# TUMFTM/ORB_SLAM3_RGBL

Hardware: AMD Instinct MI355X
Metric: RGB-L front-end frames/sec (extract+depth+match) (higher is better)
Workload: dtype u8; 1 GPU; KITTI-00 RGB-L cfg2 (synthetic stand-in); nfeatures=2000, levels=8, lidar_points=121600, match=Hamming brute force, frame i vs i+1, upsampling=InverseDilation Diamond 5, inputs=resident in HBM, parallelism=frames/sequences sharded, 1 rank(s), gather=none

## Files before the change

### orb_slam3_rgbl_amd/csrc/extractor.hip

```cpp
#include <math.h>
#include <stdarg.h>
#include <stdlib.h>
#include <string.h>

#include <algorithm>
#include <vector>

#include "brief_pattern.h"
#include "extractor_kernels.h"
#include "octree_labels.h"

namespace rgbl {

static thread_local char g_err[512] = "";
void set_error(const char* fmt, ...) {
  va_list ap;
  va_start(ap, fmt);
  vsnprintf(g_err, sizeof(g_err), fmt, ap);
  va_end(ap);
}
const char* last_error() { return g_err; }

static inline int round_even_f(float v) { return (int)lrintf(v); }
static inline int round_even_d(double v) { return (int)lrint(v); }
// ... 111 lines not shown
    t.a0 = (int16_t)round_even_f((1.f - f) * 2048);
    t.a1 = (int16_t)round_even_f(f * 2048);
    tab.push_back(t);
  }
}

int build_geometry(rgbl_extractor* e) {
  const rgbl_extractor_cfg& c = e->cfg;
  const int L = c.nlevels;
  e->L = L;
  e->scale.assign(L, 1.f); e->sigma2.assign(L, 1.f); e->inv_scale.assign(L, 1.f); e->inv_sigma2.assign(L, 1.f);
  for (int i = 1; i < L; ++i) {
    e->scale[i] = e->scale[i - 1] * c.scale_factor;
    e->sigma2[i] = e->scale[i] * e->scale[i];
  }
  for (int i = 0; i < L; ++i) {
    e->inv_scale[i] = 1.0f / e->scale[i];
    e->inv_sigma2[i] = 1.0f / e->sigma2[i];
  }
  e->per_level.assign(L, 0);
  const float factor = 1.0f / c.scale_factor;
  float desired = c.nfeatures * (1 - factor) / (1 - (float)pow((double)factor, (double)L));
  int sum = 0;
  for (int l = 0; l < L - 1; ++l) {
    e->per_level[l] = round_even_f(desired);
    sum += e->per_level[l];
    desired *= factor;
  }
  e->per_level[L - 1] = std::max(c.nfeatures - sum, 0);
  {
    int* u = e->umax.v;
    for (int i = 0; i < 16; ++i) u[i] = 0;
    const int vmax = floor_f(15 * sqrtf(2.f) / 2 + 1), vmin = ceil_f(15 * sqrtf(2.f) / 2);
    for (int v = 0; v <= vmax; ++v) u[v] = round_even_d(sqrt(225.0 - v * v));
    for (int v = 15, v0 = 0; v >= vmin; --v) {
      while (u[v0] == u[v0 + 1]) ++v0;
      u[v] = v0;
      ++v0;
    }
  }
  e->geom.assign(L, LevelGeom());
  size_t img_off = 0, slot_off = 0, node_off = 0, rootx_off = 0, xtab_off = 0, ytab_off = 0;
  int cell_off = 0, koff = 0;
  e->img_pitch = (int)align_up(c.width, 64);
  e->img_frame = (size_t)e->img_pitch * c.height;
  int tile_off = 0;
  for (int l = 0; l < L; ++l) {
    LevelGeom& g = e->geom[l];
    memset(&g, 0, sizeof(g));
    g.w = round_even_f((float)c.width * e->inv_scale[l]);
    g.h = round_even_f((float)c.height * e->inv_scale[l]);
    g.pitch = (int)align_up(g.w, 64);
    g.img_off = (uint32_t)img_off;
    img_off += (size_t)g.pitch * g.h;
    g.quota = e->per_level[l];
    g.scale = e->scale[l];
    g.patch_size = (int)(31 * e->scale[l]);
    g.max_bx = g.w - 19 + 3;
    g.max_by = g.h - 19 + 3;
    const float width = (float)(g.max_bx - kMinBorder), height = (float)(g.max_by - kMinBorder);
    g.n_cols = (int)(width / 35.f);
    g.n_rows = (int)(height / 35.f);
    if (g.n_cols < 1 || g.n_rows < 1) {
      set_error("level %d (%dx%d) is smaller than one 35-px detection cell; the reference divides by zero here", l, g.w, g.h);
      return RGBL_ERR_INVALID;
    }
    g.w_cell = (int)ceilf(width / g.n_cols);
    g.h_cell = (int)ceilf(height / g.n_rows);
    if (g.w_cell > kCellMax || g.h_cell > kCellMax) {
      set_error("cell %dx%d exceeds the kernel tile", g.w_cell, g.h_cell);
      return RGBL_ERR_INVALID;
    }
    e->max_cell = std::max(e->max_cell, std::max(g.w_cell, g.h_cell));
    e->max_cell_w = std::max(e->max_cell_w, g.w_cell);
    g.n_cells = g.n_cols * g.n_rows;
    g.m_wcell = (0x100000u + (uint32_t)g.w_cell - 1u) / (uint32_t)g.w_cell;
    g.m_hcell = (0x100000u + (uint32_t)g.h_cell - 1u) / (uint32_t)g.h_cell;
    g.cell_off = cell_off;
    cell_off += g.n_cells;
    g.cell_cap = ((g.w_cell + 1) / 2) * ((g.h_cell + 1) / 2);
    g.slot_off = (uint32_t)slot_off;
    g.key_off = (uint32_t)slot_off;
    g.key_cap = (uint32_t)((size_t)g.n_cells * g.cell_cap);
    slot_off += (size_t)g.n_cells * g.cell_cap;
    g.n_ini = (int)roundf((float)(g.max_bx - kMinBorder) / (float)(g.max_by - kMinBorder));
    if (g.n_ini < 1 || g.n_ini > kMaxRoots) {
      set_error("aspect ratio gives %d quad-tree roots (supported 1..%d; the reference fails for portrait images)", g.n_ini, kMaxRoots);
      return RGBL_ERR_INVALID;
    }
    const float hX = (float)(g.max_bx - kMinBorder) / g.n_ini;
    for (int i = 0; i <= g.n_ini; ++i) g.root_x[i] = (int)(hX * (float)i);
    g.rootx_off = (uint32_t)rootx_off;
    rootx_off += align_up((size_t)(g.max_bx - kMinBorder) + 1, 16);
    g.kcap = std::max(g.quota, 4 * g.n_ini) + 8;
    g.koff = koff;
    koff += g.kcap;
    g.node_cap = (uint32_t)g.kcap + 16;
    if (g.node_cap > 65535u) {
      set_error("nfeatures too large: level %d would need %u quad-tree nodes (limit 65535)", l, g.node_cap);
      return RGBL_ERR_INVALID;
    }
    g.node_off = (uint32_t)node_off;
    node_off += g.node_cap;
    g.xtab_off = (uint32_t)xtab_off;
    g.ytab_off = (uint32_t)ytab_off;
    if (l > 0) { xtab_off += align_up(g.w, 4); ytab_off += g.h; }
    e->blur_tiles.tile_off[l] = tile_off;
// ... 304 lines not shown
      RGBL_HIP(hipStreamWaitEvent(ls, e->ev_r, 0));
      launch_fast(ls, cells0, e->geom[k].cell_off);
      launch_octree(ls, 1, k);
      RGBL_HIP(hipEventRecord(e->ev_fb, ls));
      for (int l = k; l < L; ++l) launch_resize(s, l);
      RGBL_HIP(hipEventRecord(e->ev_pyr, s));
      launch_fast(s, e->geom[k].cell_off, e->cells_frame);
      launch_octree(s, k, L);
      RGBL_HIP(hipStreamWaitEvent(bs, e->ev_pyr, 0));
      launch_gauss(bs, tiles0, e->blur_tiles.tile_off[L]);
      RGBL_HIP(hipEventRecord(e->ev_blur, bs));
      RGBL_HIP(hipStreamWaitEvent(s, e->ev_fb, 0));
      RGBL_HIP(hipStreamWaitEvent(s, e->ev_fast0, 0));
      RGBL_HIP(hipStreamWaitEvent(s, e->ev_blur, 0));
    } else {
    if (overlap) {
      RGBL_HIP(hipEventRecord(e->ev_start, s));
      RGBL_HIP(hipStreamWaitEvent(bs, e->ev_start, 0));
      launch_fast(bs, 0, cells0);
      launch_gauss(bs, 0, tiles0);
      launch_octree(bs, 0, 1);
      RGBL_HIP(hipEventRecord(e->ev_fast0, bs));
    }
    for (int l = 1; l < L; ++l) launch_resize(s, l);
    if (overlap) {
      RGBL_HIP(hipEventRecord(e->ev_pyr, s));
      RGBL_HIP(hipStreamWaitEvent(bs, e->ev_pyr, 0));
      launch_gauss(bs, tiles0, e->blur_tiles.tile_off[L]);
      RGBL_HIP(hipEventRecord(e->ev_blur, bs));
    } else {
      launch_gauss(s, 0, e->blur_tiles.tile_off[L]);
    }
    if (overlap) {
      launch_fast(s, cells0, e->cells_frame);
    } else {
      launch_fast(s, 0, e->cells_frame);
    }
    if (overlap) {
      launch_octree(s, 1, L);
      RGBL_HIP(hipStreamWaitEvent(s, e->ev_fast0, 0));
    } else {
      launch_octree(s, 0, L);
    }
    if (overlap) RGBL_HIP(hipStreamWaitEvent(s, e->ev_blur, 0));
    }
  }
  const bool lapping = lap1 >= 19 && lap1 >= lap0;
  rgbl_keypoint* kp_dst = lapping ? e->d_tmp_kp : d_kp;
  uint8_t* desc_dst = lapping ? e->d_tmp_desc : d_desc;
  int lap_cap = cap;
  if (lapping) lap_cap = std::min(cap, e->out_cap);
  const bool split_desc = !e->timer.enabled && batch >= 8 && L > 1 && e->geom[1].koff > 0;
  const int slot_split = split_desc ? e->geom[1].koff : 0;
  auto launch_desc = [&](hipStream_t st, int slot_begin, int slot_end, int write_total) {
    if (slot_end <= slot_begin) return;
    e->timer.begin("k_orient_brief", st);
    hipLaunchKernelGGL(k_orient_brief<256>, xcd_grid(e->xcd_map, (slot_end - slot_begin + 4 * kKpPerWave - 1) / (4 * kKpPerWave), batch), dim3(256), 0, st, e->d_geom, L, e->umax,
                       e->d_pattern, d_imgs, stride, frame_stride, e->d_pyr, e->pyr_frame, e->d_blur, e->pyr_frame,
                       e->d_kpkey, e->d_kpcount, (size_t)e->kp_frame, kp_dst, desc_dst, lapping ? e->out_cap : cap, d_n,
                       lapping ? (int32_t*)nullptr : d_mono, e->d_err, slot_begin, slot_end, write_total);
    e->timer.end(st);
  };
  if (split_desc) {
    launch_desc(e->aux_stream, 0, slot_split, 0);
    RGBL_HIP(hipEventRecord(e->ev_desc0, e->aux_stream));
  }
  launch_desc(s, slot_split, e->kp_frame, 1);
  if (split_desc) RGBL_HIP(hipStreamWaitEvent(s, e->ev_desc0, 0));
  if (lapping) {
    (void)lap_cap;
    if (cap < e->out_cap) {
      set_error("vLappingArea packing needs cap >= %d", e->out_cap);
      return RGBL_ERR_CAPACITY;
    }
    e->timer.begin("k_lapping_permute", s);
    hipLaunchKernelGGL(k_lapping_permute, dim3(batch), dim3(256), 0, s, e->d_tmp_kp, e->d_tmp_desc, e->out_cap, d_kp,
                       d_desc, cap, d_n, (float)lap0, (float)lap1, d_mono);
    e->timer.end(s);
  }
  RGBL_HIP(hipGetLastError());
  e->dense_dirty = false;
  return RGBL_OK;
}

int check_device_flags(rgbl_extractor* e) {
  int flags = 0;
  RGBL_HIP(hipMemcpy(&flags, e->d_err, sizeof(int), hipMemcpyDeviceToHost));
  if (flags) {
    RGBL_HIP(hipMemset(e->d_err, 0, sizeof(int)));
    RGBL_HIP(hipMemset(e->d_levelcnt, 0, sizeof(uint32_t) * (size_t)e->cfg.max_batch * e->L));
    if (flags & 3) { set_error("quad-tree scratch overflow (flags=%d)", flags); return RGBL_ERR_OVERFLOW; }
    set_error("more keypoints than the caller's capacity");
    return RGBL_ERR_CAPACITY;
  }
  return RGBL_OK;
}

}

extern "C" {

const char* rgbl_last_error(void) { return rgbl::last_error(); }
const char* rgbl_backend(void) {
#ifdef RGBL_EMU
  return "emu";
#else
  return "hip:gfx950";
#endif
}
int rgbl_device_count(void) {
  int n = 0;
  if (hipGetDeviceCount(&n) != hipSuccess) return 0;
  return n;
// ... 422 lines not shown
  return RGBL_OK;
}

int rgbl_extract_color(rgbl_extractor* e, const uint8_t* img, int channels, int blue_first, int w, int h, int stride, int lap0,
                       int lap1, rgbl_keypoint* out_kp, uint8_t* out_desc, int cap, int* out_n, int* out_mono,
                       uint8_t* out_gray, int gray_stride) {
  if (out_n) *out_n = 0;
  if (out_mono) *out_mono = -1;
  if (!e) { set_error("null handle"); return RGBL_ERR_INVALID; }
  if (!img || w <= 0 || h <= 0) { set_error("empty image"); return RGBL_ERR_EMPTY; }
  if (!out_kp || !out_desc || !out_n || !out_mono) { set_error("null output"); return RGBL_ERR_INVALID; }
  if (channels == 1) {
    if (out_gray) for (int y = 0; y < h; ++y) memcpy(out_gray + (size_t)y * gray_stride, img + (size_t)y * stride, w);
    return rgbl_extract(e, img, w, h, stride, lap0, lap1, out_kp, out_desc, cap, out_n, out_mono);
  }
  if ((channels != 3 && channels != 4) || w != e->cfg.width || h != e->cfg.height || stride < w * channels || cap < 1 ||
      (out_gray && gray_stride < w)) {
    set_error("colour image %dx%dx%d does not match the handle (%dx%d)", w, h, channels, e->cfg.width, e->cfg.height);
    return RGBL_ERR_INVALID;
  }
  RGBL_HIP(hipSetDevice(e->device));
  RGBL_TRY(drop_pending(e));
  hipStream_t s = e->stream;
  const size_t need = (size_t)stride * h + 16;
  if (need > e->color_bytes) {
    if (e->d_color) RGBL_HIP(hipFree(e->d_color));
    e->d_color = nullptr; e->color_bytes = 0;
    RGBL_HIP(hipMalloc(&e->d_color, need));
    e->color_bytes = need;
  }
  RGBL_HIP(hipMemcpyAsync(e->d_color, img, (size_t)(h - 1) * stride + (size_t)w * channels, hipMemcpyHostToDevice, s));
  RGBL_TRY(enqueue_cvt_gray(e, (const uint8_t*)e->d_color, 1, channels, blue_first, w, h, stride, 0, e->d_img, e->img_pitch, 0));
  if (out_gray) RGBL_HIP(hipMemcpy2DAsync(out_gray, gray_stride, e->d_img, e->img_pitch, w, h, hipMemcpyDeviceToHost, s));
  return run_staged(e, 1, e->img_pitch, lap0, lap1, out_kp, out_desc, cap, out_n, out_mono);
}

int rgbl_extractor_level_size(const rgbl_extractor* e, int level, int* w, int* h) {
  if (!e || level < 0 || level >= e->L) { set_error("bad level"); return RGBL_ERR_INVALID; }
  if (w) *w = e->geom[level].w;
  if (h) *h = e->geom[level].h;
  return RGBL_OK;
}

int rgbl_extractor_get_level(rgbl_extractor* e, int frame, int level, int blurred, int with_border, uint8_t* dst,
                             int dst_stride) {
  if (!e || !dst || level < 0 || level >= e->L || frame < 0 || frame >= e->last_batch) {
    set_error("bad level/frame");
    return RGBL_ERR_INVALID;
  }
  RGBL_HIP(hipSetDevice(e->device));
  const LevelGeom& g = e->geom[level];
  const uint8_t* src;
  int pitch;
  if (blurred) { src = e->d_blur + (size_t)frame * e->pyr_frame + g.img_off; pitch = g.pitch; }
  else if (level == 0) { src = e->last_img0 + (size_t)frame * e->last_frame0; pitch = e->last_pitch0; }
  else { src = e->d_pyr + (size_t)frame * e->pyr_frame + g.img_off; pitch = g.pitch; }
  const int border = (with_border && !blurred) ? 19 : 0;
  RGBL_HIP(hipStreamSynchronize(e->stream));
  uint8_t* inner = dst + (size_t)border * dst_stride + border;
  {
    std::vector<uint8_t> tmp((size_t)pitch * (g.h - 1) + g.w);
    RGBL_HIP(hipMemcpyAsync(tmp.data(), src, tmp.size(), hipMemcpyDeviceToHost, e->stream));
    RGBL_HIP(hipStreamSynchronize(e->stream));
    for (int y = 0; y < g.h; ++y) memcpy(inner + (size_t)y * dst_stride, tmp.data() + (size_t)y * pitch, g.w);
  }
  if (border) {
    auto refl = [](int p, int len) { while (p < 0 || p >= len) p = p < 0 ? -p : 2 * (len - 1) - p; return p; };
    for (int y = 0; y < g.h; ++y) {
      uint8_t* row = inner + (size_t)y * dst_stride;
      for (int x = 1; x <= border; ++x) { row[-x] = row[refl(-x, g.w)]; row[g.w - 1 + x] = row[refl(g.w - 1 + x, g.w)]; }
    }
    for (int y = 1; y <= border; ++y) {
      memcpy(inner + (ptrdiff_t)(-y) * dst_stride - border, inner + (ptrdiff_t)refl(-y, g.h) * dst_stride - border, g.w + 2 * border);
      memcpy(inner + (ptrdiff_t)(g.h - 1 + y) * dst_stride - border, inner + (ptrdiff_t)refl(g.h - 1 + y, g.h) * dst_stride - border,
             g.w + 2 * border);
    }
  }
  return RGBL_OK;
}

int rgbl_extractor_get_candidates(rgbl_extractor* e, int frame, int level, rgbl_keypoint* out, int cap, int* out_n) {
  if (!e || level < 0 || level >= e->L || frame < 0 || frame >= e->last_batch || !out_n) {
    set_error("bad level/frame");
    return RGBL_ERR_INVALID;
  }
  RGBL_HIP(hipSetDevice(e->device));
  RGBL_HIP(hipStreamSynchronize(e->stream));
  const LevelGeom& g = e->geom[level];
  auto emit = [&](uint32_t key, int n) {
    if (out && n < cap) {
      rgbl_keypoint kp;
      kp.x = (float)(key & 0xfff); kp.y = (float)((key >> 12) & 0xfff); kp.size = 7.f; kp.angle = -1.f;
      kp.response = (float)(key >> 24); kp.octave = 0; kp.class_id = -1;
      out[n] = kp;
    }
  };
  int n = 0;
  if (e->dense) {
    uint32_t C = 0;
    RGBL_HIP(hipMemcpy(&C, e->d_levelcnt + ((size_t)e->cfg.max_batch + frame) * e->L + level, sizeof(uint32_t), hipMemcpyDeviceToHost));
    C = std::min(C, g.key_cap);
    std::vector<uint32_t> keys(C);
    if (C) RGBL_HIP(hipMemcpy(keys.data(), e->d_keys_a + (size_t)frame * e->keys_frame + g.key_off, sizeof(uint32_t) * C, hipMemcpyDeviceToHost));
    auto order = [&](uint32_t key) {
      const uint32_t x = (key & 0xfff) - 3u, y = ((key >> 12) & 0xfff) - 3u;
      const uint32_t col = x / (uint32_t)g.w_cell, row = y / (uint32_t)g.h_cell;
      return ((unsigned long long)(row * (uint32_t)g.n_cols + col) << 14) | ((y - row * g.h_cell) << 7) | (x - col * g.w_cell);
    };
// ... 297 lines not shown
```

### orb_slam3_rgbl_amd/csrc/extractor_kernels.h

```cpp
#pragma once
#include "common.h"
#include "sincos_glibc.h"

namespace rgbl {

constexpr int kMaxLevels = 16;
constexpr int kMaxRoots = 16;
constexpr int kMinBorder = 16;

struct ResizeTab {
  int32_t sofs;
  int16_t a0, a1;
};

struct LevelGeom {
  int w, h, pitch;
  uint32_t img_off;
  int quota;
  int kcap, koff;
  int n_cols, n_rows, w_cell, h_cell, max_bx, max_by;
  int n_cells, cell_off, cell_cap;
  uint32_t slot_off;
  uint32_t key_off, key_cap;
  uint32_t node_off, node_cap;
  int n_ini;
  int root_x[kMaxRoots + 1];
  int root_first[kMaxRoots + 1];
  uint32_t m_wcell, m_hcell;
  uint32_t rootx_off;
  uint32_t xtab_off, ytab_off;
  float scale;
  int patch_size;
};

struct UMax { int v[16]; };

struct QNode {
  uint16_t x0, x1, y0, y1;
  uint32_t beg;
  uint32_t cnt;
};
struct QDiv { uint32_t c[4]; };

__device__ __forceinline__ uint32_t pack_key(int x, int y, int s) { return (uint32_t)x | ((uint32_t)y << 12) | ((uint32_t)s << 24); }
__device__ __forceinline__ int key_x(uint32_t k) { return (int)(k & 0xfff); }
__device__ __forceinline__ int key_y(uint32_t k) { return (int)((k >> 12) & 0xfff); }
__device__ __forceinline__ int key_s(uint32_t k) { return (int)(k >> 24); }

__device__ __forceinline__ uint32_t load_u32_unaligned(const uint8_t* p) {
  uint32_t v;
  __builtin_memcpy(&v, p, 4);
  return v;
}

constexpr int kResizeRows = 4;
constexpr int kResizeLanes = 32, kResizeWG = kResizeLanes * 4;
struct ResizeGroup { uint32_t sel[4], w[4]; };
static_assert(sizeof(ResizeGroup) == 32, "two 16-byte loads per group");

__global__ __launch_bounds__(kResizeWG) void k_resize_linear(const uint8_t* __restrict__ src, int spitch,
                                                       size_t sframe, int sw, int sh,
                                                       uint8_t* __restrict__ dst, int dpitch, size_t dframe,
                                                       int dw, int dh, const ResizeTab* __restrict__ xtab,
                                                       const ResizeGroup* __restrict__ xgroups, const int32_t* __restrict__ xsxa,
                                                       const ResizeTab* __restrict__ ytab, int tiles_x) {
  const int tx = threadIdx.x % kResizeLanes, ty = threadIdx.x / kResizeLanes;
  const int tile_y = xcd_item() / tiles_x, tile_x = xcd_item() - tile_y * tiles_x;
  const int dx0 = (tile_x * kResizeLanes + tx) * 4;
  const int dy0 = (tile_y * 4 + ty) * kResizeRows;
  if (dy0 >= dh || dx0 >= dw) return;
  const uint8_t* S = src + (size_t)xcd_frame() * sframe;
  uint8_t* D = dst + (size_t)xcd_frame() * dframe + (size_t)dy0 * dpitch;
  const int sxa = xsxa[dx0 >> 2];
  const uint4* g4 = reinterpret_cast<const uint4*>(xgroups + (dx0 >> 2));
  const uint4 gs = g4[0], gw = g4[1];
  ResizeTab ry[kResizeRows];
#pragma unroll
  for (int r = 0; r < kResizeRows; ++r) ry[r] = ytab[imin(dy0 + r, dh - 1)];
  if (sxa >= 0) {
    uint32_t r0l[kResizeRows], r0h[kResizeRows], r1l[kResizeRows], r1h[kResizeRows];
#pragma unroll
    for (int r = 0; r < kResizeRows; ++r) {
      const int sy0 = imin(imax(ry[r].sofs, 0), sh - 1), sy1 = imin(imax(ry[r].sofs + 1, 0), sh - 1);
      const uint8_t* S0 = S + (size_t)sy0 * spitch + sxa;
      const uint8_t* S1 = S + (size_t)sy1 * spitch + sxa;
      r0l[r] = load_u32_unaligned(S0); r0h[r] = load_u32_unaligned(S0 + 4);
      r1l[r] = load_u32_unaligned(S1); r1h[r] = load_u32_unaligned(S1 + 4);
    }
// ... 467 lines not shown
  if (active) {
    out_mul[i] = mul24(av & 0xffffffu, b);
    out_add[i] = add_flag((int)av, m);
  }
  if (i < n && (lane_id() % 5) != 4) lds_dma16(src + (size_t)16 * i + (i & 3), s_buf + wave_id() * 1024);
  __syncthreads();
  if (i < n)
    for (int k = 0; k < 16; ++k) out_dma[(size_t)16 * i + k] = s_buf[16 * tid + k];
}

struct CellGroup { uint32_t first, count; };
constexpr int kCompactCells = 256;

__global__ __launch_bounds__(256) void k_compact_cells(const CellGroup* __restrict__ groups, const FastCell* __restrict__ cells,
                                                        const uint32_t* __restrict__ cell_cnt, size_t cells_frame,
                                                        const uint32_t* __restrict__ slots, size_t slots_frame,
                                                        const LevelGeom* __restrict__ geom, int n_levels,
                                                        uint32_t* __restrict__ dense_keys, size_t keys_frame,
                                                        uint32_t* __restrict__ level_cnt, int group_begin) {
  __shared__ uint32_t s_pref[kCompactCells + 1];
  __shared__ uint32_t s_scan[8];
  __shared__ uint32_t s_base;
  const int tid = threadIdx.x, f = xcd_frame();
  const CellGroup G = groups[xcd_item() + group_begin];
  const FastCell first = cells[G.first];
  const uint32_t cnt = tid < (int)G.count ? cell_cnt[(size_t)f * cells_frame + G.first + tid] : 0u;
  uint32_t total;
  const uint32_t ex = block_exclusive_scan<uint32_t>(cnt, s_scan, &total);
  s_pref[tid] = ex;
  if (tid == 0) {
    s_pref[kCompactCells] = total;
    s_base = total ? atomicAdd(&level_cnt[(size_t)f * n_levels + first.l], total) : 0u;
  }
  __syncthreads();
  if (total == 0) return;
  const uint32_t* src = slots + (size_t)f * slots_frame + first.slot_base;
  uint32_t* out = dense_keys + (size_t)f * keys_frame + geom[first.l].key_off + s_base;
  const uint32_t cell_cap = first.cell_cap;
  for (uint32_t i = (uint32_t)tid; i < total; i += 256u) {
    uint32_t lo = 0;
#pragma unroll
    for (uint32_t step = kCompactCells / 2; step >= 1; step >>= 1)
      if (s_pref[lo + step] <= i) lo += step;
    out[i] = src[lo * cell_cap + (i - s_pref[lo])];
  }
}

constexpr int kBlurTW = 128, kBlurTH = 32;
struct BlurTiles { int tile_off[kMaxLevels + 1]; int tiles_x[kMaxLevels]; };

struct GaussTile { uint16_t x0, y0, w, h, pitch; uint8_t l, pad; uint32_t img_off; };
static_assert(sizeof(GaussTile) == 16, "one s_load_dwordx4 per tile");

template <int BS>
__global__ __launch_bounds__(BS) void k_gauss7(const GaussTile* __restrict__ tiles,
                                                    const uint8_t* __restrict__ img0, int pitch0, size_t frame0,
                                                    const uint8_t* __restrict__ pyr, size_t pyr_frame,
                                                    uint8_t* __restrict__ blur, size_t blur_frame, int tile_begin) {
  constexpr int kPairs = (kBlurTH + 6) / 2;
  __shared__ uint32_t s_p[kPairs * kBlurTW];
  const int f = xcd_frame();
  const int tid = threadIdx.x, bx = xcd_item() + tile_begin;
  const GaussTile T = tiles[bx];
  const int x0 = T.x0, y0 = T.y0;
  const uint8_t* img = (T.l == 0) ? img0 + (size_t)f * frame0 : pyr + (size_t)f * pyr_frame + T.img_off;
  const int pitch = (T.l == 0) ? pitch0 : (int)T.pitch;
  const int W = T.w, H = T.h;
  const uint32_t kWA = 18u | (34u << 8) | (48u << 16) | (56u << 24), kWB = 48u | (34u << 8) | (18u << 16);

  auto h_sums = [&](const uint32_t (&w)[2][3], int j, int cg) {
    uint32_t hs[2][4];
#pragma unroll
    for (int rr = 0; rr < 2; ++rr) {
#pragma unroll
      for (int i = 0; i < 4; ++i) {
        const uint32_t lo = i == 3 ? w[rr][1] : align_bytes(w[rr][1], w[rr][0], i + 1);
        const uint32_t hi = i == 3 ? w[rr][2] : align_bytes(w[rr][2], w[rr][1], i + 1);
        hs[rr][i] = udot4(lo, kWA, udot4(hi, kWB, 0u));
      }
    }
    uint4 v;
    v.x = hs[0][0] | (hs[1][0] << 16); v.y = hs[0][1] | (hs[1][1] << 16);
    v.z = hs[0][2] | (hs[1][2] << 16); v.w = hs[0][3] | (hs[1][3] << 16);
    *reinterpret_cast<uint4*>(&s_p[j * kBlurTW + 4 * cg]) = v;
  };
  const bool rows_inside = y0 >= 3 && y0 + kBlurTH + 3 <= H;
  for (int task = tid; task < kPairs * 32; task += BS) {
    const int j = task >> 5, cg = task & 31;
    const int x = x0 + 4 * cg;
    if (x < 4 || x + 8 > W) continue;
    int ya = y0 + 2 * j - 3, yb = ya + 1;
    if (!rows_inside) { ya = reflect101(ya, H); yb = reflect101(yb, H); }
    const uint8_t* row0 = img + __umul24((uint32_t)ya, (uint32_t)pitch) + x;
    const uint8_t* row1 = img + __umul24((uint32_t)yb, (uint32_t)pitch) + x;
    uint32_t w[2][3];
    w[0][0] = load_u32_unaligned(row0 - 4); w[0][1] = load_u32_unaligned(row0); w[0][2] = load_u32_unaligned(row0 + 4);
    w[1][0] = load_u32_unaligned(row1 - 4); w[1][1] = load_u32_unaligned(row1); w[1][2] = load_u32_unaligned(row1 + 4);
    h_sums(w, j, cg);
  }
  {
    const int cg_last = imin(31, (W - 1 - x0) >> 2);
    const int cg_r0 = imax(0, imin(cg_last + 1, ((W - 8 - x0) >> 2) + 1));
    const int n_right = (x0 + 4 * cg_r0 + 8 > W) ? cg_last - cg_r0 + 1 : 0;
    const int n_left = (x0 == 0 && cg_r0 > 0) ? 1 : 0;
    const int n_edge = n_left + n_right;
    for (int task = tid; task < kPairs * n_edge; task += BS) {
      const int j = task / n_edge, e = task - j * n_edge;
      const int cg = e < n_left ? 0 : cg_r0 + (e - n_left);
      const int x = x0 + 4 * cg;
      uint32_t w[2][3];
#pragma unroll
      for (int rr = 0; rr < 2; ++rr) {
        const uint8_t* row = img + __umul24((uint32_t)reflect101(y0 + 2 * j + rr - 3, H), (uint32_t)pitch);
        w[rr][0] = w[rr][1] = w[rr][2] = 0;
#pragma unroll
        for (int k = 0; k < 4; ++k) {
          w[rr][0] |= (uint32_t)row[reflect101(x - 4 + k, W)] << (8 * k);
          w[rr][1] |= (uint32_t)row[reflect101(x + k, W)] << (8 * k);
          w[rr][2] |= (uint32_t)row[reflect101(x + 4 + k, W)] << (8 * k);
        }
      }
      h_sums(w, j, cg);
    }
  }
  __syncthreads();
  for (int item = tid; item < 256; item += BS) {
  const int cg = item & 31, rg = item >> 5;
  const int x = x0 + 4 * cg;
  if (x >= W) continue;
  uint32_t pv[5][4];
#pragma unroll
  for (int j = 0; j < 5; ++j) {
    const uint4 v = *reinterpret_cast<const uint4*>(&s_p[(2 * rg + j) * kBlurTW + 4 * cg]);
    pv[j][0] = v.x; pv[j][1] = v.y; pv[j][2] = v.z; pv[j][3] = v.w;
  }
  const uint32_t kE0 = 18u | (34u << 16), kE1 = 48u | (56u << 16), kE2 = 48u | (34u << 16), kE3 = 18u;
  const uint32_t kO0 = 18u << 16, kO1 = 34u | (48u << 16), kO2 = 56u | (48u << 16), kO3 = 34u | (18u << 16);
  uint8_t* D = blur + (size_t)f * blur_frame + T.img_off + (__umul24((uint32_t)(y0 + 4 * rg), (uint32_t)T.pitch) + (uint32_t)x);
#pragma unroll
  for (int o = 0; o < 4; ++o) {
    if (y0 + 4 * rg + o >= H) break;
    const int b = o >> 1;
    uint32_t out = 0;
#pragma unroll
    for (int i = 0; i < 4; ++i) {
      uint32_t acc = 32768u;
      if ((o & 1) == 0) {
        acc = udot2(pv[b][i], kE0, acc); acc = udot2(pv[b + 1][i], kE1, acc);
        acc = udot2(pv[b + 2][i], kE2, acc); acc = udot2(pv[b + 3][i], kE3, acc);
      } else {
        acc = udot2(pv[b][i], kO0, acc); acc = udot2(pv[b + 1][i], kO1, acc);
        acc = udot2(pv[b + 2][i], kO2, acc); acc = udot2(pv[b + 3][i], kO3, acc);
      }
      out = i == 0 ? acc >> 16 : perm_bytes(acc, out, i == 1 ? 0x0c0c0600u : i == 2 ? 0x0c060100u : 0x06020100u);
    }
    *reinterpret_cast<uint32_t*>(D + __umul24((uint32_t)o, (uint32_t)T.pitch)) = out;
  }
  }
}

struct SortPair { uint64_t k; uint32_t v; };
struct SortView {
  uint64_t* key; uint32_t* val;
  __host__ __device__ SortPair get(int i) const { SortPair p; p.k = key[i]; p.v = val[i]; return p; }
  __host__ __device__ void set(int i, SortPair p) const { key[i] = p.k; val[i] = p.v; }
  __host__ __device__ void swap(int i, int j) const { SortPair a = get(i), b = get(j); set(i, b); set(j, a); }
  __host__ __device__ bool less(int i, int j) const { return key[i] < key[j]; }
};
__host__ __device__ inline void ss_push_heap(const SortView& a, int first, int hole, int top, SortPair value) {
  int parent = (hole - 1) / 2;
  while (hole > top && a.key[first + parent] < value.k) {
    a.set(first + hole, a.get(first + parent));
    hole = parent;
    parent = (hole - 1) / 2;
  }
  a.set(first + hole, value);
}
__host__ __device__ inline void ss_adjust_heap(const SortView& a, int first, int hole, int len, SortPair value) {
  const int top = hole;
  int child = hole;
  while (child < (len - 1) / 2) {
    child = 2 * (child + 1);
    if (a.less(first + child, first + child - 1)) --child;
    a.set(first + hole, a.get(first + child));
    hole = child;
  }
  if ((len & 1) == 0 && child == (len - 2) / 2) {
    child = 2 * (child + 1);
    a.set(first + hole, a.get(first + child - 1));
    hole = child - 1;
  }
  ss_push_heap(a, first, hole, top, value);
}
__host__ __device__ inline void ss_heap_sort(const SortView& a, int first, int last) {
  const int len = last - first;
  if (len >= 2) {
    int parent = (len - 2) / 2;
    for (;;) {
      SortPair v = a.get(first + parent);
      ss_adjust_heap(a, first, parent, len, v);
      if (parent == 0) break;
      --parent;
    }
  }
  while (last - first > 1) {
    --last;
    SortPair v = a.get(last);
    a.set(last, a.get(first));
    ss_adjust_heap(a, first, 0, last - first, v);
  }
// ... 695 lines not shown
  }

  RGBL_STAMP(4);
  uint32_t* out = b.kp_key + (size_t)f * b.kp_frame + g.koff;
  if (n > g.kcap) { if (tid == 0) atomicOr(b.err, 2); n = g.kcap; }
  for (int pos = tid; pos < n; pos += BS) {
    const QNode nd = cur[pos];
    const uint32_t cnt = nd.cnt & 0x7fffffffu;
    const uint32_t* src = ((nd.cnt >> 31) ? keys_b : keys_a) + nd.beg;
    uint32_t best = src[0];
    for (uint32_t k = 1; k < cnt; ++k) {
      const uint32_t key = src[k];
      if (key_s(key) > key_s(best)) best = key;
    }
    out[pos] = best;
  }
  if (tid == 0) b.kp_count[(size_t)f * n_levels + l] = n;
  RGBL_STAMP(5);
  if (b.dbg && tid == 0) { b.dbg[((size_t)f * n_levels + l) * 16 + 6] = C; b.dbg[((size_t)f * n_levels + l) * 16 + 7] = (unsigned long long)n; }
}

__device__ __forceinline__ float fast_atan2_deg(float y, float x) {
  const float scale = (float)(180.0 / 3.14159265358979323846);
  const float p1 = 0.9997878412794807f * scale, p3 = -0.3258083974640975f * scale,
              p5 = 0.1555786518463281f * scale, p7 = -0.04432655554792128f * scale;
  const float eps = (float)2.2204460492503131e-16;
  const float ax = fabsf(x), ay = fabsf(y);
  float a, c, c2;
  if (ax >= ay) {
    c = __fdiv_rn(ay, ax + eps);
    c2 = c * c;
    a = (((p7 * c2 + p5) * c2 + p3) * c2 + p1) * c;
  } else {
    c = __fdiv_rn(ax, ay + eps);
    c2 = c * c;
    a = 90.f - (((p7 * c2 + p5) * c2 + p3) * c2 + p1) * c;
  }
  if (x < 0) a = 180.f - a;
  if (y < 0) a = 360.f - a;
  return a;
}

constexpr int kKpPerWave = 8;

__device__ __forceinline__ int bcast_i(int v, int k) {
#ifdef RGBL_EMU
  return __shfl(v, k);
#else
  return __builtin_amdgcn_readlane(v, k);
#endif
}
__device__ __forceinline__ float bcast_f(float v, int k) { return __int_as_float(bcast_i(__float_as_int(v), k)); }

template <int BS>
__global__ __launch_bounds__(BS) void k_orient_brief(const LevelGeom* __restrict__ geom, int n_levels, UMax umax,
                                                      const int8_t* __restrict__ pattern,
                                                      const uint8_t* __restrict__ img0, int pitch0, size_t frame0,
                                                      const uint8_t* __restrict__ pyr, size_t pyr_frame,
                                                      const uint8_t* __restrict__ blur, size_t blur_frame,
                                                      const uint32_t* __restrict__ kp_key,
                                                      const int* __restrict__ kp_count, size_t kp_frame,
                                                      rgbl_keypoint* __restrict__ out_kp,
                                                      uint8_t* __restrict__ out_desc, int cap,
                                                      int32_t* __restrict__ out_n, int32_t* __restrict__ out_mono,
                                                      int* __restrict__ err, int slot_begin, int slot_end, int write_total) {
  __shared__ unsigned long long s_patch_q[BS / 64][37 * 5];
  const int lane = lane_id(), wave = wave_id();
  const int bx = xcd_item(), f = xcd_frame();
  const int* cnts = kp_count + (size_t)f * n_levels;

  const int s0 = slot_begin + (bx * (BS / 64) + wave) * kKpPerWave;
  const int slot = s0 + (lane < kKpPerWave ? lane : 0);
  int l = 0;
  for (int j = 1; j < n_levels; ++j) l += (slot >= geom[j].koff) ? 1 : 0;
  const int idx = slot - geom[l].koff;
  bool valid = lane < kKpPerWave && slot < slot_end && idx < cnts[l];
  int dense = idx;
  for (int j = 0; j < n_levels; ++j) dense += (j < l) ? cnts[j] : 0;
  if (write_total && bx == 0 && wave == 0 && lane == 0) {
    int total = 0;
    for (int j = 0; j < n_levels; ++j) total += cnts[j];
    out_n[f] = total < cap ? total : cap;
    if (out_mono) out_mono[f] = total < cap ? total : cap;
    if (total > cap) atomicOr(err, 4);
  }
  if (valid && dense >= cap) valid = false;
  const uint32_t key = valid ? kp_key[(size_t)f * kp_frame + slot] : 0u;
  const int kx = key_x(key) + kMinBorder, ky = key_y(key) + kMinBorder;
  const unsigned long long vmask = __ballot(valid);

  f32x2 px[4], py[4];
#pragma unroll
  for (int k = 0; k < 4; ++k) {
    const uint32_t pw = reinterpret_cast<const uint32_t*>(pattern)[k * 64 + lane];
    px[k] = f32x2{(float)(int8_t)(pw & 0xff), (float)(int8_t)((pw >> 16) & 0xff)};
    py[k] = f32x2{(float)(int8_t)((pw >> 8) & 0xff), (float)(int8_t)(pw >> 24)};
  }

  uint32_t rawreg[kKpPerWave][4];
  unsigned long long blreg[kKpPerWave][3];
#pragma unroll
  for (int k = 0; k < kKpPerWave; ++k) {
    if (!((vmask >> k) & 1)) continue;
    const int lk = bcast_i(l, k), x = bcast_i(kx, k), y = bcast_i(ky, k);
    const LevelGeom& g = geom[lk];
    const uint8_t* img = (lk == 0) ? img0 + (size_t)f * frame0 : pyr + (size_t)f * pyr_frame + g.img_off;
    const int pitch = (lk == 0) ? pitch0 : g.pitch;
    const uint8_t* src = img + (size_t)(y - 15) * pitch + (x - 15);
    uint4 q;
    q.x = q.y = q.z = q.w = 0u;
    if (lane < 62) __builtin_memcpy(&q, src + (__umul24((uint32_t)(lane >> 1), (uint32_t)pitch) + (uint32_t)(16 * (lane & 1))), 16);
    rawreg[k][0] = q.x; rawreg[k][1] = q.y; rawreg[k][2] = q.z; rawreg[k][3] = q.w;
  }
#pragma unroll
  for (int k = 0; k < kKpPerWave; ++k) {
    if (!((vmask >> k) & 1)) continue;
    const int lk = bcast_i(l, k), x = bcast_i(kx, k), y = bcast_i(ky, k);
    const LevelGeom& g = geom[lk];
    const uint8_t* bl = blur + (size_t)f * blur_frame + g.img_off + (size_t)(y - 18) * g.pitch + (x - 18);
#pragma unroll
    for (int j = 0; j < 3; ++j) {
      const int i = lane + 64 * j;
      const int r = i / 5, c = i - r * 5;
      unsigned long long v = 0ull;
      if (i < 37 * 5) __builtin_memcpy(&v, bl + (__umul24((uint32_t)r, (uint32_t)g.pitch) + (uint32_t)(8 * c)), 8);
      blreg[k][j] = v;
    }
  }

  uint32_t ic_mask[4] = {0u, 0u, 0u, 0u}, ic_coef[4];
  int ic_off;
  {
    const int v = (lane >> 1) - 15, half = lane & 1;
    const int d = umax.v[lane < 62 ? (v < 0 ? -v : v) : 0];
#pragma unroll
    for (int q = 0; q < 16; ++q) {
      const bool in = lane < 62 && (half ? (q + 1 <= d) : (15 - q <= d));
      ic_mask[q >> 2] |= in ? (0xffu << (8 * (q & 3))) : 0u;
    }
#pragma unroll
    for (int j = 0; j < 4; ++j) ic_coef[j] = 0x03020100u + 0x04040404u * (uint32_t)j + (half ? 0x01010101u : 0u);
    ic_off = half ? 0 : 15;
  }
  int my_m10 = 0, my_m01 = 0;
#pragma unroll
  for (int k = 0; k < kKpPerWave; ++k) {
    if (!((vmask >> k) & 1)) continue;
    uint32_t sum0 = 0, sum1 = 0;
#pragma unroll
    for (int j = 0; j < 4; ++j) {
      const uint32_t wm = rawreg[k][j] & ic_mask[j];
      sum0 = udot4(wm, 0x01010101u, sum0);
      sum1 = udot4(wm, ic_coef[j], sum1);
    }
    int m10 = (int)sum1 - ic_off * (int)sum0;
    int m01 = ((lane >> 1) - 15) * (int)sum0;
    m10 = wave_sum_uniform(m10);
    m01 = wave_sum_uniform(m01);
    if (lane == k) { my_m10 = m10; my_m01 = m01; }
  }

  __shared__ int s_mom[BS / 64 * kKpPerWave][2];
  __shared__ float s_angle[BS / 64 * kKpPerWave], s_cos[BS / 64 * kKpPerWave], s_sin[BS / 64 * kKpPerWave];
  if (lane < kKpPerWave) { s_mom[wave * kKpPerWave + lane][0] = my_m10; s_mom[wave * kKpPerWave + lane][1] = my_m01; }
  __syncthreads();
  if (wave == 0 && lane < BS / 64 * kKpPerWave) {
    const float an = fast_atan2_deg((float)s_mom[lane][1], (float)s_mom[lane][0]);
    const float factor_pi = (float)(3.14159265358979323846 / 180.f);
    const float rad = an * factor_pi;
    s_angle[lane] = an; s_cos[lane] = glibc_cosf(rad); s_sin[lane] = glibc_sinf(rad);
  }
  __syncthreads();
  const int mine = wave * kKpPerWave + (lane < kKpPerWave ? lane : 0);
  const float angle = s_angle[mine], ca = s_cos[mine], sb = s_sin[mine];

  const uint8_t* patch = reinterpret_cast<const uint8_t*>(s_patch_q[wave]);
#pragma unroll
  for (int k = 0; k < kKpPerWave; ++k) {
    if (!((vmask >> k) & 1)) continue;
    const int dk = bcast_i(dense, k);
    const float a = bcast_f(ca, k), b = bcast_f(sb, k);
    wave_sync();
#pragma unroll
    for (int j = 0; j < 3; ++j)
      if (lane + 64 * j < 37 * 5) s_patch_q[wave][lane + 64 * j] = blreg[k][j];
    wave_sync();
    const f32x2 av = {a, a}, bv = {b, b}, magic = {12582912.0f, 12582912.0f};
    constexpr int kBias = 0x400000 * 40 + 0x4B400000;
    unsigned long long bits[4];
#pragma unroll
    for (int q = 0; q < 4; ++q) {
      const f32x2 rx = px[q] * av - py[q] * bv;
      const f32x2 ry = px[q] * bv + py[q] * av;
      const f32x2 cx = rx + magic, cy = ry + magic;
      const int i0 = __mul24(__float_as_int(cy[0]), 40) + __float_as_int(cx[0]) - kBias;
      const int i1 = __mul24(__float_as_int(cy[1]), 40) + __float_as_int(cx[1]) - kBias;
      const int t0 = patch[18 * 40 + 18 + i0];
      const int t1 = patch[18 * 40 + 18 + i1];
      bits[q] = __ballot(t0 < t1);
    }
    if (lane < 4) {
      unsigned long long* d = reinterpret_cast<unsigned long long*>(out_desc + ((size_t)f * cap + dk) * 32);
      d[lane] = bits[lane];
    }
  }
  if (valid) {
    const LevelGeom& g = geom[l];
    rgbl_keypoint kp;
    kp.x = (float)kx; kp.y = (float)ky;
    if (l != 0) { kp.x = kp.x * g.scale; kp.y = kp.y * g.scale; }
    kp.size = (float)g.patch_size;
    kp.angle = angle;
    kp.response = (float)key_s(key);
    kp.octave = l;
    kp.class_id = -1;
    out_kp[(size_t)f * cap + dense] = kp;
  }
}

__global__ __launch_bounds__(256) void k_lapping_permute(const rgbl_keypoint* __restrict__ in_kp,
                                                         const uint8_t* __restrict__ in_desc, int in_cap,
                                                         rgbl_keypoint* __restrict__ out_kp,
                                                         uint8_t* __restrict__ out_desc, int cap,
                                                         const int32_t* __restrict__ n_per_frame, float lap0,
                                                         float lap1, int32_t* __restrict__ out_mono) {
  __shared__ uint32_t s_scan[8];
  const int tid = threadIdx.x, f = blockIdx.x;
  const int n = n_per_frame[f];
  uint32_t carry = 0;
  for (int i0 = 0; i0 < n; i0 += 256) {
    const int i = i0 + tid;
    rgbl_keypoint kp;
    kp.x = 0;
    uint32_t in_lap = 0;
    if (i < n) {
      kp = in_kp[(size_t)f * in_cap + i];
      in_lap = (kp.x >= lap0 && kp.x <= lap1) ? 1u : 0u;
    }
    uint32_t tot;
    const uint32_t before = carry + block_exclusive_scan<uint32_t>(in_lap, s_scan, &tot);
    carry += tot;
    if (i < n) {
      const int dst = in_lap ? (n - 1 - (int)before) : (i - (int)before);
      out_kp[(size_t)f * cap + dst] = kp;
      const uint4* s = reinterpret_cast<const uint4*>(in_desc + ((size_t)f * in_cap + i) * 32);
      uint4* d = reinterpret_cast<uint4*>(out_desc + ((size_t)f * cap + dst) * 32);
      d[0] = s[0];
      d[1] = s[1];
    }
  }
  if (tid == 0) out_mono[f] = n - (int)carry;
}

__global__ __launch_bounds__(kOctWide) void k_test_block_sort(uint64_t* key, uint32_t* val, int n) {
  __shared__ unsigned long long s_skey_pad[kSortLds + 8];
  __shared__ uint16_t s_seg_first[kSortLds], s_seg_last[kSortLds];
  __shared__ SortRanges s_ra, s_rb;
  __shared__ int s_sort_cnt[2];
  uint64_t* w = reinterpret_cast<uint64_t*>(s_skey_pad + 4);
  for (int i = threadIdx.x; i < n; i += kOctWide) w[i] = (key[i] << 16) | (val[i] & 0xffffu);
  __syncthreads();
  block_sort_restated<kOctWide>(w, n, s_seg_first, s_seg_last, &s_ra, &s_rb, s_sort_cnt);
  for (int i = threadIdx.x; i < n; i += kOctWide) { key[i] = w[i] >> 16; val[i] = (uint32_t)(w[i] & 0xffffu); }
}

struct ScaleTables { float scale[kMaxLevels], inv_scale[kMaxLevels]; };
struct PyrView { const uint8_t* img0; int pitch0; size_t frame0; const uint8_t* pyr; size_t pyr_frame; };
constexpr int kStereoTile = 2048;
constexpr int kStereoLanes = 4;
constexpr int kStereoBatch = 16;
constexpr int kStereoRowBias = 4096;
// ... 334 lines not shown
```

Measured before the change: 145,500 frames/s.

## Store blurred pyramid in 32x4 tiled layout for line-local BRIEF patch loads

The Gaussian blur kernel now writes its output in a tiled layout where each 128-byte line holds a 32x4 block. It uses quad DPP exchanges to transpose four rows into 16-byte stores. The orientation/BRIEF kernel reads 8-byte aligned patch pieces through the tiled addressing, using six pieces per row and a 48-byte shared pitch, so a patch touches fewer cache lines. The change also adds optional clock-stamp instrumentation behind a macro, and host readback of blurred levels untiles the data. The costs are extra address arithmetic, one more patch load per lane, and padded blur rows.

```diff
diff --git a/orb_slam3_rgbl_amd/csrc/extractor.hip b/orb_slam3_rgbl_amd/csrc/extractor.hip
--- a/orb_slam3_rgbl_amd/csrc/extractor.hip
+++ b/orb_slam3_rgbl_amd/csrc/extractor.hip
@@ -187,7 +187,7 @@
     g.h = round_even_f((float)c.height * e->inv_scale[l]);
     g.pitch = (int)align_up(g.w, 64);
     g.img_off = (uint32_t)img_off;
-    img_off += (size_t)g.pitch * g.h;
+    img_off += (size_t)g.pitch * blur_rows(g.h);
     g.quota = e->per_level[l];
     g.scale = e->scale[l];
     g.patch_size = (int)(31 * e->scale[l]);
@@ -598,13 +598,18 @@
   if (lapping) lap_cap = std::min(cap, e->out_cap);
   const bool split_desc = !e->timer.enabled && batch >= 8 && L > 1 && e->geom[1].koff > 0;
   const int slot_split = split_desc ? e->geom[1].koff : 0;
+#ifdef RGBL_ORIENT_STAMPS
+#define RGBL_OB_DBG_ARG , e->d_dbg
+#else
+#define RGBL_OB_DBG_ARG
+#endif
   auto launch_desc = [&](hipStream_t st, int slot_begin, int slot_end, int write_total) {
     if (slot_end <= slot_begin) return;
     e->timer.begin("k_orient_brief", st);
     hipLaunchKernelGGL(k_orient_brief<256>, xcd_grid(e->xcd_map, (slot_end - slot_begin + 4 * kKpPerWave - 1) / (4 * kKpPerWave), batch), dim3(256), 0, st, e->d_geom, L, e->umax,
                        e->d_pattern, d_imgs, stride, frame_stride, e->d_pyr, e->pyr_frame, e->d_blur, e->pyr_frame,
                        e->d_kpkey, e->d_kpcount, (size_t)e->kp_frame, kp_dst, desc_dst, lapping ? e->out_cap : cap, d_n,
-                       lapping ? (int32_t*)nullptr : d_mono, e->d_err, slot_begin, slot_end, write_total);
+                       lapping ? (int32_t*)nullptr : d_mono, e->d_err, slot_begin, slot_end, write_total RGBL_OB_DBG_ARG);
     e->timer.end(st);
   };
   if (split_desc) {
@@ -1133,8 +1138,17 @@
   const LevelGeom& g = e->geom[level];
   const uint8_t* src;
   int pitch;
-  if (blurred) { src = e->d_blur + (size_t)frame * e->pyr_frame + g.img_off; pitch = g.pitch; }
-  else if (level == 0) { src = e->last_img0 + (size_t)frame * e->last_frame0; pitch = e->last_pitch0; }
+  if (blurred) {
+    std::vector<uint8_t> tmp((size_t)g.pitch * blur_rows(g.h));
+    RGBL_HIP(hipStreamSynchronize(e->stream));
+    RGBL_HIP(hipMemcpyAsync(tmp.data(), e->d_blur + (size_t)frame * e->pyr_frame + g.img_off, tmp.size(), hipMemcpyDeviceToHost, e->stream));
+    RGBL_HIP(hipStreamSynchronize(e->stream));
+    for (int y = 0; y < g.h; ++y)
+      for (int x = 0; x < g.w; x += kBlurTileW)
+        memcpy(dst + (size_t)y * dst_stride + x, tmp.data() + blur_offset(x, y, g.pitch), std::min(kBlurTileW, g.w - x));
+    return RGBL_OK;
+  }
+  if (level == 0) { src = e->last_img0 + (size_t)frame * e->last_frame0; pitch = e->last_pitch0; }
   else { src = e->d_pyr + (size_t)frame * e->pyr_frame + g.img_off; pitch = g.pitch; }
   const int border = (with_border && !blurred) ? 19 : 0;
   RGBL_HIP(hipStreamSynchronize(e->stream));
diff --git a/orb_slam3_rgbl_amd/csrc/extractor_kernels.h b/orb_slam3_rgbl_amd/csrc/extractor_kernels.h
--- a/orb_slam3_rgbl_amd/csrc/extractor_kernels.h
+++ b/orb_slam3_rgbl_amd/csrc/extractor_kernels.h
@@ -34,6 +34,15 @@
 };
 
 struct UMax { int v[16]; };
+
+constexpr int kBlurTileWLog = 5, kBlurTileHLog = 2;
+constexpr int kBlurTileW = 1 << kBlurTileWLog, kBlurTileH = 1 << kBlurTileHLog;
+static_assert(kBlurTileW * kBlurTileH == 128 && kBlurTileW >= 16 && kBlurTileH >= 4, "one line per tile; k_gauss7 stores 16-byte row pieces of 4-row blocks");
+__host__ __device__ inline uint32_t blur_rows(int h) { return (uint32_t)(h + kBlurTileH - 1) & ~(uint32_t)(kBlurTileH - 1); }
+__host__ __device__ inline uint32_t blur_offset(int x, int y, int pitch) {
+  return (uint32_t)(y >> kBlurTileHLog) * (uint32_t)(kBlurTileH * pitch) + ((uint32_t)(x >> kBlurTileWLog) << 7) +
+         ((uint32_t)(y & (kBlurTileH - 1)) << kBlurTileWLog) + (uint32_t)(x & (kBlurTileW - 1));
+}
 
 struct QNode {
   uint16_t x0, x1, y0, y1;
@@ -607,6 +616,15 @@
 struct GaussTile { uint16_t x0, y0, w, h, pitch; uint8_t l, pad; uint32_t img_off; };
 static_assert(sizeof(GaussTile) == 16, "one s_load_dwordx4 per tile");
 
+template <int kBit>
+__device__ __forceinline__ uint32_t quad_xchg(uint32_t v) {
+#ifdef RGBL_EMU
+  return (uint32_t)__shfl_xor((int)v, kBit);
+#else
+  return (uint32_t)__builtin_amdgcn_update_dpp(0, (int)v, kBit == 1 ? 0xB1 : 0x4E, 0xF, 0xF, false);
+#endif
+}
+
 template <int BS>
 __global__ __launch_bounds__(BS) void k_gauss7(const GaussTile* __restrict__ tiles,
                                                     const uint8_t* __restrict__ img0, int pitch0, size_t frame0,
@@ -681,8 +699,6 @@
   __syncthreads();
   for (int item = tid; item < 256; item += BS) {
   const int cg = item & 31, rg = item >> 5;
-  const int x = x0 + 4 * cg;
-  if (x >= W) continue;
   uint32_t pv[5][4];
 #pragma unroll
   for (int j = 0; j < 5; ++j) {
@@ -691,12 +707,11 @@
   }
   const uint32_t kE0 = 18u | (34u << 16), kE1 = 48u | (56u << 16), kE2 = 48u | (34u << 16), kE3 = 18u;
   const uint32_t kO0 = 18u << 16, kO1 = 34u | (48u << 16), kO2 = 56u | (48u << 16), kO3 = 34u | (18u << 16);
-  uint8_t* D = blur + (size_t)f * blur_frame + T.img_off + (__umul24((uint32_t)(y0 + 4 * rg), (uint32_t)T.pitch) + (uint32_t)x);
+  uint32_t out[4];
 #pragma unroll
   for (int o = 0; o < 4; ++o) {
-    if (y0 + 4 * rg + o >= H) break;
     const int b = o >> 1;
-    uint32_t out = 0;
+    out[o] = 0;
 #pragma unroll
     for (int i = 0; i < 4; ++i) {
       uint32_t acc = 32768u;
@@ -707,10 +722,23 @@
         acc = udot2(pv[b][i], kO0, acc); acc = udot2(pv[b + 1][i], kO1, acc);
         acc = udot2(pv[b + 2][i], kO2, acc); acc = udot2(pv[b + 3][i], kO3, acc);
       }
-      out = i == 0 ? acc >> 16 : perm_bytes(acc, out, i == 1 ? 0x0c0c0600u : i == 2 ? 0x0c060100u : 0x06020100u);
-    }
-    *reinterpret_cast<uint32_t*>(D + __umul24((uint32_t)o, (uint32_t)T.pitch)) = out;
-  }
+      out[o] = i == 0 ? acc >> 16 : perm_bytes(acc, out[o], i == 1 ? 0x0c0c0600u : i == 2 ? 0x0c060100u : 0x06020100u);
+    }
+  }
+  const int q = cg & 3;
+#pragma unroll
+  for (int o = 0; o < 4; o += 2) {
+    const uint32_t got = quad_xchg<1>((q & 1) ? out[o] : out[o + 1]);
+    if (q & 1) out[o] = got; else out[o + 1] = got;
+  }
+#pragma unroll
+  for (int o = 0; o < 2; ++o) {
+    const uint32_t got = quad_xchg<2>((q & 2) ? out[o] : out[o + 2]);
+    if (q & 2) out[o] = got; else out[o + 2] = got;
+  }
+  const int x = x0 + 16 * (cg >> 2), y = y0 + 4 * rg + q;
+  if (x < W && y < H)
+    *reinterpret_cast<uint4*>(blur + (size_t)f * blur_frame + T.img_off + blur_offset(x, y, T.pitch)) = make_uint4(out[0], out[1], out[2], out[3]);
   }
 }
 
@@ -1512,6 +1540,13 @@
 }
 __device__ __forceinline__ float bcast_f(float v, int k) { return __int_as_float(bcast_i(__float_as_int(v), k)); }
 
+#ifdef RGBL_ORIENT_STAMPS
+#define RGBL_OB_DBG_PARAM , unsigned long long* __restrict__ dbg
+#define RGBL_OB_STAMP(k) const unsigned long long ob_t##k = rgbl_clock()
+#else
+#define RGBL_OB_DBG_PARAM
+#define RGBL_OB_STAMP(k) do { } while (0)
+#endif
 template <int BS>
 __global__ __launch_bounds__(BS) void k_orient_brief(const LevelGeom* __restrict__ geom, int n_levels, UMax umax,
                                                       const int8_t* __restrict__ pattern,
@@ -1523,8 +1558,10 @@
                                                       rgbl_keypoint* __restrict__ out_kp,
                                                       uint8_t* __restrict__ out_desc, int cap,
                                                       int32_t* __restrict__ out_n, int32_t* __restrict__ out_mono,
-                                                      int* __restrict__ err, int slot_begin, int slot_end, int write_total) {
-  __shared__ unsigned long long s_patch_q[BS / 64][37 * 5];
+                                                      int* __restrict__ err, int slot_begin, int slot_end, int write_total RGBL_OB_DBG_PARAM) {
+  RGBL_OB_STAMP(0);
+  constexpr int kPatchPieces = 6, kPatchPitch = 8 * kPatchPieces, kPatchLoads = (37 * kPatchPieces + 63) / 64;
+  __shared__ unsigned long long s_patch_q[BS / 64][37 * kPatchPieces];
   const int lane = lane_id(), wave = wave_id();
   const int bx = xcd_item(), f = xcd_frame();
   const int* cnts = kp_count + (size_t)f * n_levels;
@@ -1558,7 +1595,7 @@
   }
 
   uint32_t rawreg[kKpPerWave][4];
-  unsigned long long blreg[kKpPerWave][3];
+  unsigned long long blreg[kKpPerWave][kPatchLoads];
 #pragma unroll
   for (int k = 0; k < kKpPerWave; ++k) {
     if (!((vmask >> k) & 1)) continue;
@@ -1577,17 +1614,19 @@
     if (!((vmask >> k) & 1)) continue;
     const int lk = bcast_i(l, k), x = bcast_i(kx, k), y = bcast_i(ky, k);
     const LevelGeom& g = geom[lk];
-    const uint8_t* bl = blur + (size_t)f * blur_frame + g.img_off + (size_t)(y - 18) * g.pitch + (x - 18);
-#pragma unroll
-    for (int j = 0; j < 3; ++j) {
+    const uint8_t* bl = blur + (size_t)f * blur_frame + g.img_off;
+    const int xa = (x - 18) & ~7, pitch = g.pitch;
+#pragma unroll
+    for (int j = 0; j < kPatchLoads; ++j) {
       const int i = lane + 64 * j;
-      const int r = i / 5, c = i - r * 5;
+      const int r = i / kPatchPieces, c = i - r * kPatchPieces;
       unsigned long long v = 0ull;
-      if (i < 37 * 5) __builtin_memcpy(&v, bl + (__umul24((uint32_t)r, (uint32_t)g.pitch) + (uint32_t)(8 * c)), 8);
+      if (i < 37 * kPatchPieces) __builtin_memcpy(&v, bl + blur_offset(xa + 8 * c, y - 18 + r, pitch), 8);
       blreg[k][j] = v;
     }
   }
 
+  RGBL_OB_STAMP(1);
   uint32_t ic_mask[4] = {0u, 0u, 0u, 0u}, ic_coef[4];
   int ic_off;
   {
@@ -1618,7 +1657,11 @@
     m10 = wave_sum_uniform(m10);
     m01 = wave_sum_uniform(m01);
     if (lane == k) { my_m10 = m10; my_m01 = m01; }
-  }
+#ifdef RGBL_ORIENT_STAMPS
+    if (k == __builtin_ctzll(vmask | (1ull << 63)) && lane == 0) atomicAdd(&dbg[1], rgbl_clock() - ob_t1);
+#endif
+  }
+  RGBL_OB_STAMP(2);
 
   __shared__ int s_mom[BS / 64 * kKpPerWave][2];
   __shared__ float s_angle[BS / 64 * kKpPerWave], s_cos[BS / 64 * kKpPerWave], s_sin[BS / 64 * kKpPerWave];
@@ -1633,6 +1676,7 @@
   __syncthreads();
   const int mine = wave * kKpPerWave + (lane < kKpPerWave ? lane : 0);
   const float angle = s_angle[mine], ca = s_cos[mine], sb = s_sin[mine];
+  RGBL_OB_STAMP(3);
 
   const uint8_t* patch = reinterpret_cast<const uint8_t*>(s_patch_q[wave]);
 #pragma unroll
@@ -1640,23 +1684,24 @@
     if (!((vmask >> k) & 1)) continue;
     const int dk = bcast_i(dense, k);
     const float a = bcast_f(ca, k), b = bcast_f(sb, k);
+    const int centre = 18 * kPatchPitch + 18 + ((bcast_i(kx, k) - 18) & 7);
     wave_sync();
 #pragma unroll
-    for (int j = 0; j < 3; ++j)
-      if (lane + 64 * j < 37 * 5) s_patch_q[wave][lane + 64 * j] = blreg[k][j];
+    for (int j = 0; j < kPatchLoads; ++j)
+      if (lane + 64 * j < 37 * kPatchPieces) s_patch_q[wave][lane + 64 * j] = blreg[k][j];
     wave_sync();
     const f32x2 av = {a, a}, bv = {b, b}, magic = {12582912.0f, 12582912.0f};
-    constexpr int kBias = 0x400000 * 40 + 0x4B400000;
+    constexpr int kBias = 0x400000 * kPatchPitch + 0x4B400000;
     unsigned long long bits[4];
 #pragma unroll
     for (int q = 0; q < 4; ++q) {
       const f32x2 rx = px[q] * av - py[q] * bv;
       const f32x2 ry = px[q] * bv + py[q] * av;
       const f32x2 cx = rx + magic, cy = ry + magic;
-      const int i0 = __mul24(__float_as_int(cy[0]), 40) + __float_as_int(cx[0]) - kBias;
-      const int i1 = __mul24(__float_as_int(cy[1]), 40) + __float_as_int(cx[1]) - kBias;
-      const int t0 = patch[18 * 40 + 18 + i0];
-      const int t1 = patch[18 * 40 + 18 + i1];
+      const int i0 = __mul24(__float_as_int(cy[0]), kPatchPitch) + __float_as_int(cx[0]) - kBias;
+      const int i1 = __mul24(__float_as_int(cy[1]), kPatchPitch) + __float_as_int(cx[1]) - kBias;
+      const int t0 = patch[centre + i0];
+      const int t1 = patch[centre + i1];
       bits[q] = __ballot(t0 < t1);
     }
     if (lane < 4) {
@@ -1664,6 +1709,7 @@
       d[lane] = bits[lane];
     }
   }
+  RGBL_OB_STAMP(4);
   if (valid) {
     const LevelGeom& g = geom[l];
     rgbl_keypoint kp;
@@ -1676,7 +1722,14 @@
     kp.class_id = -1;
     out_kp[(size_t)f * cap + dense] = kp;
   }
-}
+#ifdef RGBL_ORIENT_STAMPS
+  if (vmask && lane == 0) {
+    atomicAdd(&dbg[0], ob_t1 - ob_t0); atomicAdd(&dbg[2], ob_t2 - ob_t1); atomicAdd(&dbg[3], ob_t3 - ob_t2);
+    atomicAdd(&dbg[4], ob_t4 - ob_t3); atomicAdd(&dbg[5], rgbl_clock() - ob_t4); atomicAdd(&dbg[7], 1ull);
+  }
+#endif
+}
+#undef RGBL_OB_STAMP
 
 __global__ __launch_bounds__(256) void k_lapping_permute(const rgbl_keypoint* __restrict__ in_kp,
                                                          const uint8_t* __restrict__ in_desc, int in_cap,
```

Measured after the change: 149,700 frames/s (median of 6 runs). 2.9% higher.
